# krejciadam/hammock

Measured on AMD Instinct MI355X. Metric: pairwise BLOSUM62 ShiftedScorer scores/sec (all-vs-all, thresholded neighbour list), higher is better.
Workload: dtype u8 (8-bit SWAR lanes, host-proven ranges with 16-bit / literal fallbacks; scores are int32-exact)

## Files before the change

### hammock_amd/_native.py

```python
from __future__ import annotations

import ctypes as C
import os

_HERE = os.path.dirname(os.path.abspath(__file__))
LIB_PATH = os.path.join(_HERE, "lib", "libhammock_hip.so")

HMK_OK = 0
HMK_ERR_BAD_ARG = 1
HMK_ERR_SHIFT_TOO_BIG = 2
HMK_ERR_DEVICE = 3
HMK_ERR_OOM = 4
HMK_ERR_REFERENCE_WOULD_CRASH = 5
HMK_ERR_CAPACITY = 6
HMK_ERR_NO_SEQUENCES = 7
HMK_EDGE_SHARDS = 64
HMK_MAX_LEN = 32
HMK_SURVEY_MAX_BINS = 1024
HMK_PROFILE_SYMBOLS = 21
HMK_PROFILE_MAX_WIDTH = 96
HMK_TARGET_MAX_LEN = 1 << 20
HMK_SCAN_ALL_WINDOWS = 1

SYMBOLS = [
    "hmk_abi_version", "hmk_last_kernel_ms", "hmk_create", "hmk_create_multi", "hmk_device_count", "hmk_destroy", "hmk_last_error", "hmk_set_sequences",
    "hmk_score_pairs_shifted", "hmk_score_with_shift", "hmk_score_pairs_local", "hmk_score_block_shifted", "hmk_score_block_local",
    "hmk_score_pairs_global", "hmk_score_block_global", "hmk_neighbors_global", "hmk_search_global",
    "hmk_neighbors_shifted", "hmk_neighbors_local", "hmk_neighbors_shifted_dev", "hmk_compact_edges_dev", "hmk_pack_rows_dev", "hmk_unpack_rows_dev",
    "hmk_neighbors_last_plan", "hmk_neighbors_last_plan_shared", "hmk_search_shifted", "hmk_search_local", "hmk_search_best_shifted",
    "hmk_assign_shifted", "hmk_assign_local", "hmk_match_clusters_shifted", "hmk_match_clusters_local", "hmk_greedy_continue",
    "hmk_greedy_cluster", "hmk_greedy_from_edges", "hmk_greedy_from_edges_dev", "hmk_greedy_last_phases",
    "hmk_clinkage_cluster", "hmk_clinkage_from_edges", "hmk_set_java_hashset", "hmk_reserve",
    "hmk_cluster_pairs_shifted", "hmk_clinkage_merge", "hmk_clinkage_merge_from_edges",
    "hmk_cluster_linkage_shifted", "hmk_clinkage_split", "hmk_clinkage_split_from_edges",
    "hmk_components_shifted", "hmk_components_from_edges", "hmk_components_from_edges_dev",
    "hmk_cluster_align_shifted", "hmk_score_survey_shifted", "hmk_cluster_separation_shifted",
    "hmk_greedy_sweep", "hmk_greedy_sweep_from_edges", "hmk_greedy_sweep_from_edges_dev",
    "hmk_greedy_orders", "hmk_greedy_orders_from_edges",
    "hmk_representatives_shifted", "hmk_representatives_from_edges", "hmk_representatives_from_edges_dev",
    "hmk_density_shifted", "hmk_density_from_edges", "hmk_density_from_edges_dev",
    "hmk_cluster_profile", "hmk_set_targets", "hmk_scan_shifted",
]


# ... 175 lines not shown
    L.hmk_score_pairs_local.argtypes = [vp, p_u32, p_u32, u64, i32, i32, p_i32]
    L.hmk_score_pairs_global.argtypes = [vp, p_u32, p_u32, u64, i32, i32, p_i32]
    L.hmk_score_with_shift.argtypes = [vp, p_u32, p_u32, u64, i32, i32, p_i32, p_i32]
    L.hmk_score_block_shifted.argtypes = [vp, u32, u32, u32, u32, i32, i32, p_i32]
    L.hmk_score_block_local.argtypes = [vp, u32, u32, u32, u32, i32, i32, p_i32]
    L.hmk_score_block_global.argtypes = [vp, u32, u32, u32, u32, i32, i32, p_i32]
    L.hmk_neighbors_shifted.argtypes = [vp, i32, i32, i32, u32, u32, p_u64, u64, p_u64, C.POINTER(NeighborStats)]
    L.hmk_neighbors_local.argtypes = [vp, i32, i32, i32, u32, u32, p_u64, u64, p_u64, C.POINTER(NeighborStats)]
    L.hmk_neighbors_global.argtypes = [vp, i32, i32, i32, u32, u32, p_u64, u64, p_u64, C.POINTER(NeighborStats)]
    L.hmk_neighbors_shifted_dev.argtypes = [vp, i32, i32, i32, u32, u32, vp, u64, vp, vp]
    L.hmk_compact_edges_dev.argtypes = [vp, vp, u64, vp, vp, u64, vp, vp]
    L.hmk_pack_rows_dev.argtypes = [vp, vp, u64, vp, i32, vp, vp, u64, vp]
    L.hmk_unpack_rows_dev.argtypes = [vp, vp, vp, i32, vp, u64, vp]
    L.hmk_neighbors_last_plan.argtypes = [vp, C.POINTER(NeighborStats)]
    L.hmk_neighbors_last_plan_shared.argtypes = [vp, C.POINTER(C.c_uint32), C.POINTER(C.c_uint32)]
    L.hmk_search_shifted.argtypes = [vp, u32, u32, u32, u32, i32, i32, i32, p_u64, u64, p_u64, C.POINTER(NeighborStats)]
    L.hmk_search_local.argtypes = [vp, u32, u32, u32, u32, i32, i32, i32, p_u64, u64, p_u64, C.POINTER(NeighborStats)]
    L.hmk_search_global.argtypes = [vp, u32, u32, u32, u32, i32, i32, i32, p_u64, u64, p_u64, C.POINTER(NeighborStats)]
    L.hmk_search_best_shifted.argtypes = [vp, u32, u32, u32, u32, i32, i32, i32, u32, p_u32, p_i32, p_u32, C.POINTER(NeighborStats)]
    L.hmk_assign_shifted.argtypes = [vp, u32, u32, u32, u32, p_u32, p_i32, u32, i32, i32, i32, u32, p_u32, p_i32, p_u32,
                                     C.POINTER(NeighborStats)]
    L.hmk_assign_local.argtypes = [vp, u32, u32, u32, u32, p_u32, p_i32, u32, i32, i32, i32, u32, p_u32, p_i32, p_u32,
                                   C.POINTER(NeighborStats)]
    L.hmk_match_clusters_shifted.argtypes = [vp, u32, u32, p_u32, u32, u32, u32, p_u32, p_i32, u32, i32, i32, i32, u32, p_u32, p_i32, p_u32,
                                             C.POINTER(NeighborStats)]
    L.hmk_match_clusters_local.argtypes = [vp, u32, u32, p_u32, u32, u32, u32, p_u32, p_i32, u32, i32, i32, i32, u32, p_u32, p_i32, p_u32,
                                           C.POINTER(NeighborStats)]
    L.hmk_greedy_continue.argtypes = [vp, u32, u32, u32, u32, p_u32, p_i32, u32, i32, i32, i32, p_i32, p_i32, C.POINTER(ContinueStats)]
    L.hmk_greedy_cluster.argtypes = [vp, i32, i32, i32, i32, p_i32, p_i32, p_i32, C.POINTER(GreedyStats)]
    L.hmk_greedy_from_edges_dev.argtypes = [vp, vp, u64, i32, i32, p_i32, p_i32, p_i32, C.POINTER(GreedyStats)]
# ... 54 lines not shown
```

### hammock_amd/api.py

```python
from __future__ import annotations

import ctypes as C

import numpy as np

from . import _native as N

AMINO_ACIDS = "ARNDCQEGHILKMFPSTWYVBZX*"
_NAME_TO_NUM = {c: i for i, c in enumerate(AMINO_ACIDS)}


class HammockException(Exception):
    """HammockException.java"""


class DataException(HammockException):
    """DataException.java -- e.g. "Shift too big" (ShiftedScorer.java:59-62)."""


class FileFormatException(HammockException):
    """FileFormatException.java"""


class DeviceError(HammockException):
# ... 480 lines not shown
            self._raise(st)

    def last_plan(self):
        stats = N.NeighborStats()
        st = N.lib.hmk_neighbors_last_plan(self._h, C.byref(stats))
        if st:
            self._raise(st)
        return stats

    def last_plan_shared(self):
        paired, shared = C.c_uint32(0), C.c_uint32(0)
        st = N.lib.hmk_neighbors_last_plan_shared(self._h, C.byref(paired), C.byref(shared))
        if st:
            self._raise(st)
        return int(paired.value), int(shared.value)

    def greedy_cluster(self, max_shift, shift_penalty, threshold, max_clusters):
        cid = np.full(max(self.n, 1), -1, dtype=np.int32)
        order = np.full(max(self.n, 1), -1, dtype=np.int32)
        self.member_rank = np.zeros(max(self.n, 1), dtype=np.int32)
        stats = N.GreedyStats()
        st = N.lib.hmk_greedy_cluster(self._h, int(max_shift), int(shift_penalty), int(threshold), int(max_clusters),
                                      _ptr(cid, C.c_int32), _ptr(order, C.c_int32),
                                      _ptr(self.member_rank, C.c_int32), C.byref(stats))
        if st:
            self._raise(st, stats)
        return cid[:self.n], order[:stats.n_result_clusters], stats

    def reserve(self, n_sequences):
        st = N.lib.hmk_reserve(self._h, int(n_sequences))
# ... 626 lines not shown
```

### hammock_amd/csrc/hmk_api.cpp

```cpp
#include "hmk_ctx.h"

using namespace hmk::impl;

extern "C" {

int hmk_abi_version(void) { return HMK_ABI_VERSION; }

double hmk_last_kernel_ms(const hmk_ctx *ctx) { return ctx ? ctx->last_kernel_ms : 0.0; }

const char *hmk_last_error(const hmk_ctx *ctx) { return ctx ? ctx->err.c_str() : g_last_error.c_str(); }

int hmk_create(const int32_t *matrix, int device, hmk_ctx **out) {
    if (!matrix || !out) return fail(nullptr, HMK_ERR_BAD_ARG, "hmk_create: null argument");
    *out = nullptr;
    hmk_ctx *ctx = new (std::nothrow) hmk_ctx();
    if (!ctx) return fail(nullptr, HMK_ERR_OOM, "out of memory");
    std::memcpy(ctx->M, matrix, sizeof(ctx->M));
    ctx->min_m = ctx->max_m = matrix[0];
    for (int e = 0; e < 576; e++) {
        ctx->min_m = std::min(ctx->min_m, matrix[e]);
        ctx->max_m = std::max(ctx->max_m, matrix[e]);
        if (matrix[e] != matrix[(e % 24) * 24 + e / 24]) ctx->symmetric = false;
        if (matrix[e] < -1000 || matrix[e] > 1000) {
            delete ctx;
// ... 253 lines not shown
    if (!ctx->plan.valid) return fail(ctx, HMK_ERR_BAD_ARG, "no neighbour pass has been planned yet");
    *stats = ctx->plan.stats;
    return HMK_OK;
}

int hmk_neighbors_last_plan_shared(hmk_ctx *ctx, uint32_t *paired_tiles, uint32_t *run_shared_tiles) {
    if (!ctx || !paired_tiles || !run_shared_tiles) return fail(ctx, HMK_ERR_BAD_ARG, "null argument");
    std::lock_guard<std::mutex> lock(ctx->mu);
    refresh_switches(ctx);
    if (!ctx->plan.valid) return fail(ctx, HMK_ERR_BAD_ARG, "no neighbour pass has been planned yet");
    *paired_tiles = ctx->plan.paired_tiles;
    *run_shared_tiles = ctx->plan.run_shared_tiles;
    return HMK_OK;
}

int hmk_neighbors_shifted(hmk_ctx *ctx, int max_shift, int shift_penalty, int threshold, uint32_t part,
                          uint32_t n_parts, uint64_t *edges, uint64_t capacity, uint64_t *n_edges,
                          hmk_neighbor_stats *stats) {
    if (!ctx) return fail(nullptr, HMK_ERR_BAD_ARG, "null context");
    std::lock_guard<std::mutex> lock(ctx->mu);
    refresh_switches(ctx);
    if (!n_edges) return fail(ctx, HMK_ERR_BAD_ARG, "n_edges must not be null");
    unsigned long long counts[HMK_EDGE_SHARDS];
    double ms = 0;
    int st = neighbors_internal(ctx, max_shift, shift_penalty, threshold, part, n_parts, capacity, counts, &ms);
    if (st) return st;
    const uint64_t total = total_of(counts);
    *n_edges = total;
    if (stats) {
        *stats = ctx->plan.stats;
// ... 280 lines not shown
```

### hammock_amd/csrc/hmk_common.cpp

```cpp
#include <atomic>

#include "hmk_ctx.h"
#include "hmk_grid.h"

namespace hmk {

static std::atomic<int> g_test_grid_cap{0};
void set_test_grid_cap(int cap) { g_test_grid_cap.store(cap < 1 ? 0 : cap, std::memory_order_relaxed); }
uint32_t capped_grid(const char *kernel, uint32_t wanted) {
    const int cap = g_test_grid_cap.load(std::memory_order_relaxed);
    if (cap < 1 || wanted <= (uint32_t)cap) return wanted;
    std::fprintf(stderr, "[hmk grid] %s %u -> %d\n", kernel, wanted, cap);
    return (uint32_t)cap;
}

namespace impl {

thread_local std::string g_last_error;

void Switches::read() {
    auto flag = [](const char *name) { return getenv(name) != nullptr; };
    auto num = [](const char *name, int dflt) { const char *v = getenv(name); return v ? atoi(v) : dflt; };
    *this = Switches();
    greedy_timing = flag("HMK_GREEDY_TIMING");
    no_band = flag("HMK_NO_BAND");
    no_rows_kernel = flag("HMK_NO_ROWS_KERNEL");
    key_sort = flag("HMK_NO_KEY_SORT") ? 0 : num("HMK_KEY_SORT_KEYS", 2) == 1 ? 1 : 2;
    no_row_shared = flag("HMK_NO_ROW_SHARED");
    key_row_pairs = getenv("HMK_KEY_ROW_PAIRS") ? (num("HMK_KEY_ROW_PAIRS", 0) != 0 ? 1 : 0) : -1;
    no_row_run_share = flag("HMK_NO_ROW_RUN_SHARE");
    adj_8byte = flag("HMK_ADJ_8BYTE");
    local_literal = flag("HMK_LOCAL_LITERAL");
    local_signed = flag("HMK_LOCAL_SIGNED");
    local_no_pk = flag("HMK_LOCAL_NO_PK");
    multi_replicate = flag("HMK_MULTI_REPLICATE");
    multi_force_copies = flag("HMK_MULTI_FORCE_COPIES");
    if (const char *v = getenv("HMK_SECOND_LOOP")) second_loop = std::strcmp(v, "device") == 0 ? 1 : 2;
    phase1_threads = std::max(0, num("HMK_PHASE1_THREADS", 0));
    phase1_window = std::max(0, num("HMK_PHASE1_WINDOW", 0));
    if (const char *v = getenv("HMK_PHASE1_HOST_BAND")) {
        host_band_rows = std::max(0, atoi(v));
        if (const char *c = std::strchr(v, ',')) host_band_far_t = std::max(0, atoi(c + 1));
    }
    loop_chain = getenv("HMK_LOOP_CHAIN") ? (num("HMK_LOOP_CHAIN", 0) != 0 ? 1 : 0) : -1;
    loop_passes = std::min(8, std::max(0, num("HMK_LOOP_PASSES", 0)));
// ... 221 lines not shown
```

### hammock_amd/csrc/hmk_ctx.h

```cpp
#ifndef HMK_CTX_H
#define HMK_CTX_H
#include <hip/hip_runtime_api.h>

#include <algorithm>
#include <chrono>
#include <condition_variable>
#include <functional>
#include <future>
#include <memory>
#include <cstdio>
#include <cstdlib>
#include <cstring>
#include <map>
#include <mutex>
#include <numeric>
#include <string>
#include <tuple>
#include <thread>
#include <vector>

#include "hmk_internal.h"
#include "hmk_kernels.h"
#include "hmk_sizing.h"

// ... 68 lines not shown
    SB_SCAN_HITS, SB_SCAN_CNT,
    SB_SCAN_HASH, SB_SCAN_PAIRS, SB_SCAN_COV,
    SB_ORD_EDGES, SB_ORD_STATE, SB_ORD_POS,
    SB_ORD_IDS, SB_ORD_SUPPORT, SB_ORD_PARTNERS,
    SB_N
};

struct Switches {
    bool greedy_timing = false;
    bool no_band = false;
    bool no_rows_kernel = false;
    int key_sort = 2;
    bool no_row_shared = false;
    int key_row_pairs = -1;
    bool no_row_run_share = false;
    bool adj_8byte = false;
    bool local_literal = false;
    bool local_signed = false;
    bool local_no_pk = false;
    bool multi_replicate = false;
    bool multi_force_copies = false;
    int second_loop = 0;
    int phase1_threads = 0, phase1_window = 0;
    int host_band_rows = 0, host_band_far_t = 0;
    int loop_chain = -1;
    int loop_passes = 0;
    int precheck = 0;
    int late_buffers_delay_ms = 0;
    int csr_bucket_shift = 0;
    uint64_t edge_guess = 0;
// ... 14 lines not shown

struct Plan : PlanArrays {
    bool valid = false;
    int X = 0, p = 0, thr = 0;
    uint32_t part = 0, n_parts = 1;
    uint32_t band_rows = 0;
    int64_t band_req = 0;
    int lbmax = 12, lpad = 16;
    bool exact = false;
    bool rows_exact = false;
    bool no_rows_kernel = false;
    int key_sort = 2;
    bool row_shared = true;
    int key_row_pairs = -1;
    bool row_run_share = true;
    bool key_pairs = false;
    uint32_t paired_tiles = 0, run_shared_tiles = 0;
    uint32_t *d_keyrun = nullptr;
    uint32_t *d_keytab = nullptr;
    uint32_t cols_per_tile = 16384;
    uint8_t *d_mb = nullptr;
    std::vector<Group> groups;
    hmk_neighbor_stats stats{};
    uint64_t band_pairs = 0;
    uint32_t q0 = 0, q1 = 0, r0 = 0, r1 = 0;
};

struct PlanLocal : PlanArrays {
    bool valid = false;
    uint32_t part = 0, n_parts = 1;
    bool triangle = false;
    uint32_t n_tiles = 0;
// ... 272 lines not shown
```

### hammock_amd/csrc/hmk_internal.h

```cpp
#ifndef HMK_INTERNAL_H
#define HMK_INTERNAL_H

#include <stdint.h>

#include <functional>
#include <string>
#include <vector>

#include "../../include/hammock_hip.h"

namespace hmk {


enum { PATH_U8 = 0, PATH_U16 = 1, PATH_DIRECT = 2, PATH_ROWS = 3 };

struct TileClass {
    uint8_t la, lb;
    uint8_t nd;
    uint8_t case_b;
    uint8_t x;
    uint8_t path;
    uint8_t nw;
    uint8_t pad;
    int32_t g;
// ... 21 lines not shown
    uint64_t cap_per_shard;
    uint32_t n_tiles;
    uint32_t lpad;
    uint32_t symmetric;
    uint32_t row_is_m;
    uint32_t perm_identity;
    uint32_t *deg;
    uint32_t deg_m_offset;
    const uint32_t *keyrun;
    const uint32_t *keytab;
};

constexpr int KEYTAB_DWORDS = 16;
constexpr int ROWS_KEY_PAIR_GROUPS = 2;
constexpr uint32_t ROWS_RUN_SHARED = 1u << 8;
constexpr bool rows_keyed(int x, int d, int cap, bool exact, int g) { return exact && d == 0 && (g == 1 || g == ROWS_KEY_PAIR_GROUPS) && x == 3 && cap == 12; }
constexpr int rows_key_pos(int x, int l, int q) { return l / 2 - 1 + q < x ? x : l / 2 - 1 + q; }

struct Nbr {
    uint32_t m;
    int32_t s;
    uint32_t id() const { return m; }
    int32_t score() const { return s; }
};
struct NbrPacked {
    uint32_t v;
    uint32_t id() const { return v >> 8; }
    int32_t score() const { return (int32_t)(v & 0xFFu); }
};

// ... 85 lines not shown
```

### hammock_amd/csrc/hmk_kernels.h

```cpp
#ifndef HMK_KERNELS_H
#define HMK_KERNELS_H

#include <hip/hip_runtime_api.h>
#include <stdint.h>

#include "hmk_internal.h"
#include "hmk_scan.h"

namespace hmk {

int swar_rows_per_tile(int lbmax, int nw, bool exact);
int swar_lbmax_for(int lb);

hipError_t launch_neighbors_swar(int lbmax, int nw, bool exact, const NeighborParams &P,
                                 uint32_t tile_base, uint32_t n_tiles, hipStream_t s);
bool rows_kernel_available(int X, int la, int lb, bool exact);
int rows_cap_for(int lb);
int rows_per_tile_rows(int X, int d, int cap, bool exact, bool key_pairs = false);
hipError_t launch_neighbors_rows(int X, int d, int cap, bool exact, const NeighborParams &P, uint32_t tile_base,
                                 uint32_t n_tiles, bool key_pairs, hipStream_t s);
hipError_t warm_neighbors_rows_module();
hipError_t launch_rows_keytab(const uint8_t *res_sorted, uint32_t lpad, uint32_t n, const uint8_t *mb, int case_b, int X, int L,
                              const uint32_t (&cinit)[8], uint32_t *keytab, uint32_t n_groups);
hipError_t launch_neighbors_direct(const NeighborParams &P, uint32_t tile_base, uint32_t n_tiles,
                                   const int32_t *d_matrix, int max_shift, int shift_penalty, int threshold,
                                   hipStream_t s);
hipError_t launch_probe_spin(unsigned long long *when, long long ticks, hipStream_t s);
hipError_t launch_pairs(int scorer, const uint8_t *res32, const uint8_t *len, const int32_t *d_matrix,
                        const uint32_t *pi, const uint32_t *pj, uint64_t n_pairs, uint32_t r0, uint32_t c0,
                        uint32_t width, int a, int b, int32_t *out, int32_t *out_shift, hipStream_t s);

hipError_t launch_neighbors_local(int lbmax, bool enc, bool force_signed, bool force_unpacked, const NeighborParams &P, uint32_t tile_base,
                                  uint32_t n_tiles, const int32_t *d_matrix, int gap_open, int gap_extend, int threshold, hipStream_t s);

hipError_t launch_neighbors_local_literal(const NeighborParams &P, uint32_t tile_base, uint32_t n_tiles, const int32_t *d_matrix,
                                          int gap_open, int gap_extend, int threshold, hipStream_t s);

hipError_t launch_neighbors_global(int lbmax, bool literal, const NeighborParams &P, uint32_t tile_base, uint32_t n_tiles,
// ... 105 lines not shown
```

### hammock_amd/csrc/hmk_plan.cpp

```cpp
#include "hmk_ctx.h"

namespace hmk { namespace impl {

template <class T, class Cmp>
void parallel_stable_sort(std::vector<T> &v, Cmp before) {
    const size_t n = v.size();
    const unsigned hw = usable_cpus();
    size_t runs = 1;
    while (runs < 8 && runs < (hw ? hw : 1u) && n / (2 * runs) >= 32768) runs *= 2;
    if (runs == 1) { std::stable_sort(v.begin(), v.end(), before); return; }
    std::vector<size_t> cut(runs + 1);
    for (size_t r = 0; r <= runs; r++) cut[r] = n * r / runs;
    {
        std::vector<std::thread> pool;
        for (size_t r = 1; r < runs; r++) pool.emplace_back([&, r] { std::stable_sort(v.begin() + (long)cut[r], v.begin() + (long)cut[r + 1], before); });
        std::stable_sort(v.begin(), v.begin() + (long)cut[1], before);
        for (std::thread &th : pool) th.join();
    }
    std::vector<T> other(n);
    std::vector<T> *from = &v, *to = &other;
    for (size_t width = 1; width < runs; width *= 2) {
        std::vector<std::thread> pool;
        for (size_t r = 0; r < runs; r += 2 * width) {
            auto job = [&, r] {
// ... 246 lines not shown
        c.path = u16 ? PATH_U16 : PATH_U8;
        c.g = (int32_t)g;
        const int lpd = u16 ? 2 : 4, bits = u16 ? 16 : 8;
        const int ndw = (nd + lpd - 1) / lpd;
        c.nw = (uint8_t)ndw;
        for (int t = 0; t < nd; t++) c.cinit[t / lpd] |= (uint32_t)ci[t] << ((t % lpd) * bits);
    }
    *out = c;
}

int build_plan(hmk_ctx *ctx, int X, int p, int thr, uint32_t part, uint32_t n_parts, int64_t band_rows, bool key_sort_ok) {
    Plan &pl = ctx->plan;
    const int want_keys = key_sort_ok ? ctx->sw.key_sort : 0;
    if (pl.valid && pl.X == X && pl.p == p && pl.thr == thr && pl.part == part && pl.n_parts == n_parts &&
        (band_rows < 0 || pl.band_req == band_rows) && pl.no_rows_kernel == ctx->sw.no_rows_kernel && pl.key_sort == want_keys &&
        pl.row_shared == !ctx->sw.no_row_shared && pl.key_row_pairs == ctx->sw.key_row_pairs && pl.row_run_share == !ctx->sw.no_row_run_share)
        return HMK_OK;
    free_plan(pl);
    if (band_rows < 0) band_rows = 0;
    const int64_t band_req = band_rows;
    const bool plan_timing = ctx->sw.greedy_timing;
    const auto plan_t0 = std::chrono::steady_clock::now();
    auto plan_lap = [&](const char *what) {
        if (plan_timing)
            fprintf(stderr, "[hmk plan] %s at %.2f ms\n", what,
                    std::chrono::duration<double, std::milli>(std::chrono::steady_clock::now() - plan_t0).count());
    };
    const uint32_t n = ctx->n;
    if (n == 0) return fail(ctx, HMK_ERR_NO_SEQUENCES, "no sequences set (hmk_set_sequences)");
    if (X < 0) return fail(ctx, HMK_ERR_BAD_ARG, "max_shift must be >= 0");
    if (n_parts == 0 || part >= n_parts) return fail(ctx, HMK_ERR_BAD_ARG, "part must be < n_parts");
// ... 76 lines not shown
    pl.rows_exact = false;
    if (use_rows && ctx->min_len == ctx->max_len) {
        TileClass t1;
        classify(ctx, ctx->min_len, ctx->min_len, X, p, thr, &t1);
        pl.rows_exact = (t1.path == PATH_U8 || (refine && all_rows_fit)) && rows_kernel_available(X, ctx->min_len, ctx->min_len, true);
    }
    if (!use_rows && ctx->min_len == 12 && ctx->max_len == 12 && X == 3) {
        TileClass t12;
        classify(ctx, 12, 12, X, p, thr, &t12);
        pl.exact = t12.path == PATH_U8 && t12.nw == 2;
    }
    pl.key_sort = want_keys;
    pl.row_shared = !ctx->sw.no_row_shared;
    pl.key_row_pairs = ctx->sw.key_row_pairs;
    pl.row_run_share = !ctx->sw.no_row_run_share;
    std::vector<uint32_t> keyrun;
    const int L1 = ctx->min_len;
    const bool key_sorted = pl.key_sort > 0 && pl.rows_exact && !(refine && !all_rows_fit) &&
                            rows_keyed(X, 0, L1, true, rows_per_tile_rows(X, 0, L1, true) / 8) && n >= 2;
    if (key_sorted) {
        const int k0 = rows_key_pos(X, L1, 0), k1 = rows_key_pos(X, L1, 1);
        auto key_of = [&](uint32_t k) { return (uint32_t)ctx->res[ctx->off[k] + k0] * HMK_ALPHABET + ctx->res[ctx->off[k] + k1]; };
        const uint32_t b0 = band_end[L1], b1 = bucket[L1 + 1];
        std::vector<uint32_t> cnt(HMK_ALPHABET * HMK_ALPHABET + 1, 0u), sorted(perm.begin() + b0, perm.begin() + b1);
        for (uint32_t q = b0; q < b1; q++) cnt[key_of(perm[q]) + 1]++;
        for (int v = 0; v < HMK_ALPHABET * HMK_ALPHABET; v++) cnt[v + 1] += cnt[v];
        for (uint32_t q = b0; q < b1; q++) sorted[cnt[key_of(perm[q])]++] = perm[q];
        std::copy(sorted.begin(), sorted.end(), perm.begin() + b0);
        keyrun.resize(2 * (size_t)n);
        uint32_t r0 = 0, r01 = 0;
// ... 82 lines not shown
    if (key_sorted && pl.row_shared) {
        const int k0 = rows_key_pos(X, L1, 0), k1 = rows_key_pos(X, L1, 1);
        auto keys_at = [&](uint32_t q) { const uint32_t k = perm[q]; return (uint32_t)ctx->res[ctx->off[k] + k0] << 8 | ctx->res[ctx->off[k] + k1]; };
        for (Tile &t : tiles) {
            for (uint32_t g = 0; 8 * g + 8 <= t.nrows; g++) {
                bool same = true;
                for (uint32_t r = 1; r < 8 && same; r++) same = keys_at(t.row0 + 8 * g + r) == keys_at(t.row0 + 8 * g);
                if (same) t.row_shared |= 1u << g;
            }
            if (pl.key_pairs && pl.row_run_share && t.nrows == 8u * ROWS_KEY_PAIR_GROUPS && (t.row_shared & 3u) == 3u &&
                keys_at(t.row0 + 8) == keys_at(t.row0))
                t.row_shared |= ROWS_RUN_SHARED;
        }
        plan_lap("row-shared groups");
    }
    pl.paired_tiles = pl.key_pairs ? (uint32_t)tiles.size() : 0u;
    pl.run_shared_tiles = 0;
    for (const Tile &t : tiles) pl.run_shared_tiles += (t.row_shared & ROWS_RUN_SHARED) ? 1u : 0u;

    st = upload_plan(ctx, pl, perm, (size_t)pl.lpad, 16, pl.exact ? 8 : 1, classes, tiles);
    if (!st) st = upload_biased_matrix(ctx, pl);
    if (st) return st;
    if (key_sorted) {
        if (classes.size() != 1) return fail(ctx, HMK_ERR_DEVICE, "key-sorted plan with more than one class");
        const uint32_t n_groups = (n + 7) / 8;
        const size_t tab_dwords = (size_t)n_groups * 2 * HMK_ALPHABET * KEYTAB_DWORDS;
        HIPCHK(ctx, hipMalloc((void **)&pl.d_keyrun, keyrun.size() * 4));
        HIPCHK(ctx, hipMemcpy(pl.d_keyrun, keyrun.data(), keyrun.size() * 4, hipMemcpyHostToDevice));
        HIPCHK(ctx, hipMalloc((void **)&pl.d_keytab, tab_dwords * 4));
        HIPCHK(ctx, launch_rows_keytab(pl.d_res_sorted, (uint32_t)pl.lpad, n, pl.d_mb, classes.at(0).case_b, X, L1, classes.at(0).cinit, pl.d_keytab,
                                       n_groups));
        HIPCHK(ctx, hipStreamSynchronize(nullptr));
    }
    pl.X = X; pl.p = p; pl.thr = thr; pl.part = part; pl.n_parts = n_parts;
    pl.valid = true;
    plan_lap("device copies");
    return HMK_OK;
}

static int build_plan_rect(hmk_ctx *ctx, Plan &pl, int X, int p, int thr, uint32_t q0, uint32_t q1, uint32_t r0, uint32_t r1, bool tri) {
    if (pl.valid && pl.X == X && pl.p == p && pl.thr == thr && pl.q0 == q0 && pl.q1 == q1 && pl.r0 == r0 && pl.r1 == r1 &&
        pl.no_rows_kernel == ctx->sw.no_rows_kernel)
        return HMK_OK;
    free_plan(pl);
    if (tri && !ctx->symmetric) return fail(ctx, HMK_ERR_BAD_ARG, "a triangle plan needs a symmetric matrix");
    Buckets bq, br;
// ... 152 lines not shown
```

### hammock_amd/csrc/k_neighbors_rows.h

```cpp
#ifndef HMK_NEIGHBORS_ROWS_H
#define HMK_NEIGHBORS_ROWS_H
#include "hmk_device.h"

namespace hmk {

constexpr int ROWS_STAGE_CAPFORM = 320, ROWS_STAGE_EXACT = 640, ROWS_STAGE_SHORT = 1024;
constexpr int ROWS_INLOOP_MAXCELLS = 45;
constexpr int rows_cells(int x, int cap) { return cap * (2 * x + 1) - x * (x + 1); }
constexpr bool rows_inloop(int x, int cap) { return rows_cells(x, cap) > ROWS_INLOOP_MAXCELLS; }
constexpr bool rows_inloop_shape(int x, int d, int cap, bool exact) { return (exact && d > 0) || rows_inloop(x, cap); }
constexpr int rows_stage(int x, int d, int cap, bool exact) {
    return !exact ? ROWS_STAGE_CAPFORM : rows_inloop_shape(x, d, cap, exact) ? ROWS_STAGE_EXACT : ROWS_STAGE_SHORT;
}
constexpr int rows_groups(int x, int , int cap, bool exact) {
    return !exact ? 2 : rows_inloop(x, cap) ? 1 : 2;
}
constexpr bool rows_two_ended(int x, int d, int cap, bool exact, int g) { return exact && !rows_inloop_shape(x, d, cap, exact) && g == 2; }

template <typename T>
__device__ __forceinline__ T rows_table_read(uint32_t addr) {
    return *reinterpret_cast<const volatile HMK_LDS T *>((uintptr_t)addr);
}
constexpr int rows_waves(int nd, int cap, int lds_bytes, bool exact) {
    const int v = cap + 2 * nd + 36 + (exact ? 0 : 6);
// ... 586 lines not shown
    const Tile T = P.tiles[tile_base + blockIdx.x];
    const TileClass *Cp = P.classes + T.cls;
    const int la = Cp->la;
    int lbs = EXACT_LB ? CAP : (int)Cp->lb;
    const bool case_b = Cp->case_b != 0;
    const int tid = threadIdx.x;
    HMK_LDS uint32_t *stage = (HMK_LDS uint32_t *)stage_all + __builtin_amdgcn_readfirstlane(tid >> 6) * STAGE_CAP;

    constexpr bool KEYED = KEY_FORMS && rows_keyed(X, D, CAP, EXACT_LB, G);
    const bool keyed = KEYED && P.keyrun != nullptr;
    const bool rs_first = keyed && (T.row_shared & 1u) != 0;
    const uint32_t rs_groups = keyed ? T.row_shared : 0u;

    build_begin();
    const uint32_t tab_addr = lds_addr(tab);
    for (int e = tid; e < 576; e += 256) mb[e] = P.mb[e];
    for (int e = tid; e < R * 32; e += 256) {
        const int r = e >> 5, k = e & 31;
        uint8_t v = 0;
        if ((uint32_t)r < T.nrows && (uint32_t)k < P.lpad) v = P.res_sorted[(size_t)(T.row0 + r) * P.lpad + k];
        rowres[e] = v;
    }
    __syncthreads();
    for (int e = tid; e < G * (NI + NEND) * 24 * 2; e += 256) {
        const int h = e & 1, ic = e >> 1;
        const int gi = ic / 24, c = ic - gi * 24;
        const int g = gi / (NI + NEND), k = gi - g * (NI + NEND);
        int i = k < NI ? k : la - 1 - (k - NI);
        const int dst = k < NI ? S::pos_addr(g, k) : S::end_addr(g, k - NI);
        if constexpr (KEYED)
            if ((G == 1 ? rs_first : ((rs_groups >> g) & 1u) != 0) && k == S::key_pos(0) && h == 1) i = S::key_pos(1);
        uint32_t v = 0;
        if (i >= 0 && i < la) {
#pragma unroll
            for (int q = 0; q < 4; q++) {
                const int r = 8 * g + 4 * h + q;
                if ((uint32_t)r < T.nrows) {
                    const int a = rowres[r * 32 + i];
                    v |= (uint32_t)(case_b ? mb[c * 24 + a] : mb[a * 24 + c]) << (q * 8);
                }
            }
        }
        *reinterpret_cast<uint32_t *>(tab + dst + c * 8 + h * 4) = v;
    }
    __syncthreads();
    build_end();

    uint32_t ci[ND];
#pragma unroll
    for (int u = 0; u < ND; u++) ci[u] = ((Cp->cinit[u >> 2] >> ((u & 3) * 8)) & 0xFFu) * 0x01010101u;

    constexpr bool TWO = rows_two_ended(X, D, CAP, EXACT_LB, G);
    uint32_t cnt = 0;
    uint32_t cnt_hi = 0;
    const uint32_t col_end = T.col0 + T.ncols;
    const uint32_t n_batches = (T.ncols + 255) / 256;
    const bool interior = T.diag == 0 && T.ncols % 256 == 0;
    const bool prio = true;

    const uint8_t *const res_sorted = P.res_sorted;
// ... 4 lines not shown
    const uint64_t ka64 = (uint64_t)(uintptr_t)__builtin_amdgcn_kernarg_segment_ptr();
    const uint32_t ka_lo = (uint32_t)ka64, ka_hi = (uint32_t)(ka64 >> 32);
    uint32_t acc[G];
#pragma unroll
    for (int g = 0; g < G; g++) acc[g] = 0;
    static_assert(!KEYED || (G <= 2 && 2 * ND <= KEYTAB_DWORDS), "key table entry; at most two row groups per tile");
    static_assert(!KEYED || (S::body_reads(3, false) == 58 && S::body_reads(1, false) == 65 && S::body_reads(0, false) == 72), "ordinary bodies");
    static_assert(!KEYED || (S::body_reads(3, true) == 54 && S::body_reads(1, true) == 60 && S::body_reads(0, true) == 66), "row-shared bodies (and the lead of a run-shared tile)");
    static_assert(!KEYED || (S::follower_reads(3) == 48 && S::follower_reads(1) == 53 && S::follower_reads(0) == 58), "followers of a run-shared tile");
    static_assert(!KEYED || (S::run_carried_planes(3) == 6 && S::run_carried_planes(1) == 7 && S::run_carried_planes(0) == 7), "dwords a lead hands over");
    static_assert(!KEYED || (S::run_body_adds(3, 2) == 62 && S::run_body_adds(1, 2) == 69 && S::run_body_adds(0, 2) == 75 && S::run_body_adds(3, 3) == 58 &&
                             S::run_body_adds(1, 3) == 64 && S::run_body_adds(0, 3) == 68), "sums of the lead and the follower");
    const uint32_t wave = __builtin_amdgcn_readfirstlane(tid >> 6);
    const uint32_t *kt_tile = nullptr, *kr_wave = nullptr;
    if (keyed) {
        kt_tile = P.keytab + (size_t)(T.row0 >> 3) * (2 * 24 * KEYTAB_DWORDS);
        kr_wave = P.keyrun + 2 * (size_t)(T.col0 + wave * 64);
    }
    auto key_entry = [](const uint32_t *e, uint32_t (&k0)[ND], uint32_t (&k1)[ND]) {
#pragma unroll
        for (int u = 0; u + 1 < ND; u += 2) {
            const u32x4 a = rows_const_load<u32x4>(e + 2 * u);
            k0[u] = a.x; k1[u] = a.y; k0[u + 1] = a.z; k1[u + 1] = a.w;
        }
        if constexpr (ND & 1) {
            const u32x2 a = rows_const_load<u32x2>(e + 2 * (ND - 1));
            k0[ND - 1] = a.x; k1[ND - 1] = a.y;
        }
    };
    using No = std::false_type;
    using Yes = std::true_type;
// ... 12 lines not shown
                ra = rows_const_load<u32x2>(kr_wave);
                const u32x2 rb = rows_const_load<u32x2>(kr_wave + 2 * last);
                if (ra.x == rb.x) kmode = ra.y == rb.y ? 3 : 1;
            }
        }
        uint32_t off[CAP], toff[S::NT];
        S::offsets_of(words, tw, tab_addr, tab_addr, off, toff);
        const bool look = !DEFER || (bt & 3u) == 3u || bt + 1 == n_batches;
        uint32_t Pm[ND];

        if constexpr (RUNS) {
            static_assert(INLOOP && !DEFER && !TWO, "paired tiles: an in-loop shape");
            auto body = [&](auto gt, auto kt, auto rt, uint32_t (&W0)[ND], uint32_t (&W1)[ND]) __attribute__((always_inline)) {
                constexpr int g = decltype(gt)::value, KM = decltype(kt)::value;
                constexpr bool RUN = decltype(rt)::value;
                const uint32_t *const kt_group = kt_tile + (size_t)g * (2 * 24 * KEYTAB_DWORDS);
                [[maybe_unused]] const bool row_shared = (rs_groups & (1u << g)) != 0;
                uint32_t ks0[ND], ks1[ND];
                if constexpr (KM == 3) {
                    uint32_t kb0[ND], kb1[ND];
                    key_entry(kt_group + (ra.x & 31u) * KEYTAB_DWORDS, ks0, ks1);
                    key_entry(kt_group + (24 + (ra.y & 31u)) * KEYTAB_DWORDS, kb0, kb1);
#pragma unroll
                    for (int u = 0; u < ND; u++) { ks0[u] += kb0[u]; ks1[u] += kb1[u]; }
                } else if constexpr (KM == 1) {
                    key_entry(kt_group + (ra.x & 31u) * KEYTAB_DWORDS, ks0, ks1);
#pragma unroll
                    for (int u = 0; u < ND; u++) asm volatile("" : "+s"(ks0[u]), "+s"(ks1[u]));
                }
                const uint32_t (&s0)[ND] = KM != 0 ? ks0 : ci;
                const uint32_t (&s1)[ND] = KM != 0 ? ks1 : ci;
// ... 68 lines not shown
                        uint32_t W0[ND], W1[ND];
                        body(gt, kt, No{}, W0, W1);
                        hits(gt, No{}, W0, W1);
                    });
                }
            };
            if (kmode == 3) both(std::integral_constant<int, 3>{});
            else if (kmode == 1) both(std::integral_constant<int, 1>{});
            else both(std::integral_constant<int, 0>{});
        } else {
            auto one_group = [&](auto gt) {
                constexpr int g = decltype(gt)::value;
                if ((uint32_t)(8 * g) >= T.nrows) return;
                uint32_t W0[ND], W1[ND];
                if constexpr (KEYED) {
                    const uint32_t *const kt_group = kt_tile + (size_t)g * (2 * 24 * KEYTAB_DWORDS);
                    const bool row_shared = G == 1 ? rs_first : (rs_groups & (1u << g)) != 0;
                    uint32_t ks0[ND], ks1[ND];
                    if (kmode == 3) {
                        uint32_t kb0[ND], kb1[ND];
                        key_entry(kt_group + (ra.x & 31u) * KEYTAB_DWORDS, ks0, ks1);
                        key_entry(kt_group + (24 + (ra.y & 31u)) * KEYTAB_DWORDS, kb0, kb1);
#pragma unroll
                        for (int u = 0; u < ND; u++) { ks0[u] += kb0[u]; ks1[u] += kb1[u]; }
                        read_phase_begin(prio);
                        if (RUNS && (rs_groups & ROWS_RUN_SHARED) != 0) S::template accumulate_run<g, 3, (g > 0)>(off, ks0, ks1, W0, W1, Pm);
                        else if (row_shared) S::template accumulate<g, 3, true>(off, toff, lbs, ks0, ks1, W0, W1);
                        else S::template accumulate<g, 3>(off, toff, lbs, ks0, ks1, W0, W1);
                    } else if (kmode == 1) {
                        key_entry(kt_group + (ra.x & 31u) * KEYTAB_DWORDS, ks0, ks1);
#pragma unroll
// ... 131 lines not shown
```

### hammock_amd/csrc/k_neighbors_rows.hip

```cpp
#include "k_rows_shapes.h"

namespace hmk {

int rows_cap_for(int lb) { return lb <= 12 ? 12 : lb <= 16 ? 16 : lb <= 20 ? 20 : 0; }

namespace {
int rows_part_of(int X, int d, int cap, bool exact) {
    if (exact) {
#define HMK_F(PV, XV, L) if (X == XV && d == 0 && cap == L) return PV;
        HMK_ROWS_EXACT_LIST(HMK_F)
#undef HMK_F
        return -1;
    }
#define HMK_C(PV, XV, DV, CAPV) if (X == XV && d == DV && cap == CAPV) return PV;
    HMK_ROWS_CAP_LIST(HMK_C)
#undef HMK_C
    return -1;
}
}

int rows_per_tile_rows(int X, int d, int cap, bool exact, bool key_pairs) {
    if (rows_part_of(X, d, cap, exact) < 0) return 0;
    if (key_pairs) return rows_keyed(X, d, cap, exact, ROWS_KEY_PAIR_GROUPS) ? 8 * ROWS_KEY_PAIR_GROUPS : 0;
    return 8 * rows_groups(X, d, cap, exact);
// ... 25 lines not shown
    if (e >= (uint64_t)n_groups * 2 * HMK_ALPHABET * KEYTAB_DWORDS) return;
    const int d = (int)(e % KEYTAB_DWORDS), c = (int)(e / KEYTAB_DWORDS % HMK_ALPHABET), q = (int)(e / (KEYTAB_DWORDS * HMK_ALPHABET) % 2);
    const uint32_t g = (uint32_t)(e / (2 * HMK_ALPHABET * KEYTAB_DWORDS));
    const int u = d >> 1, h = d & 1, i = rows_key_pos(X, L, q) + u - X;
    uint32_t v = 0;
    if (u <= 2 * X && i >= 0 && i < L) {
        for (int t = 0; t < 4; t++) {
            const uint32_t r = 8 * g + 4 * h + t;
            if (r < n) {
                const int a = res_sorted[(size_t)r * lpad + i];
                v |= (uint32_t)(case_b ? mb[c * HMK_ALPHABET + a] : mb[a * HMK_ALPHABET + c]) << (8 * t);
            }
        }
    }
    if (q == 0 && u <= 2 * X) v += ((cinit.w[u >> 2] >> ((u & 3) * 8)) & 0xFFu) * 0x01010101u;
    keytab[e] = v;
}

hipError_t launch_rows_keytab(const uint8_t *res_sorted, uint32_t lpad, uint32_t n, const uint8_t *mb, int case_b, int X, int L,
                              const uint32_t (&cinit)[8], uint32_t *keytab, uint32_t n_groups) {
    const uint64_t total = (uint64_t)n_groups * 2 * HMK_ALPHABET * KEYTAB_DWORDS;
    if (total == 0) return hipSuccess;
    KeytabInit ci;
    for (int k = 0; k < 8; k++) ci.w[k] = cinit[k];
    hipLaunchKernelGGL(k_rows_keytab, dim3((unsigned)((total + 255) / 256)), dim3(256), 0, nullptr, res_sorted, lpad, n, mb, case_b, X, L, ci,
                       keytab, n_groups);
    return hipGetLastError();
}

}
```

### include/hammock_hip.h

```cpp
#ifndef HAMMOCK_HIP_H
#define HAMMOCK_HIP_H

#include <stdint.h>

#ifdef __cplusplus
extern "C" {
#endif

#define HMK_ABI_VERSION 4
#define HMK_ALPHABET 24
#define HMK_MAX_LEN 32
#define HMK_MAX_SEQUENCES (1u << 24)
#define HMK_EDGE_SHARDS 64

typedef enum {
    HMK_OK = 0,
    HMK_ERR_BAD_ARG = 1,
    HMK_ERR_SHIFT_TOO_BIG = 2,
    HMK_ERR_DEVICE = 3,
    HMK_ERR_OOM = 4,
    HMK_ERR_REFERENCE_WOULD_CRASH = 5,
    HMK_ERR_CAPACITY = 6,
    HMK_ERR_NO_SEQUENCES = 7
} hmk_status;
// ... 56 lines not shown
int hmk_neighbors_global(hmk_ctx *ctx, int gap_open, int gap_extend, int threshold, uint32_t part,
                         uint32_t n_parts, uint64_t *edges, uint64_t capacity, uint64_t *n_edges,
                         hmk_neighbor_stats *stats);

int hmk_neighbors_shifted_dev(hmk_ctx *ctx, int max_shift, int shift_penalty, int threshold,
                              uint32_t part, uint32_t n_parts, void *d_edges, uint64_t capacity,
                              void *d_counts, void *stream);
int hmk_compact_edges_dev(hmk_ctx *ctx, const void *d_edges, uint64_t capacity, const void *d_counts,
                          void *d_out, uint64_t out_capacity, void *d_total, void *stream);
int hmk_pack_rows_dev(hmk_ctx *ctx, const void *d_edges, uint64_t capacity, const void *d_counts, int threshold,
                      void *d_row_start, void *d_adj, uint64_t adj_capacity, void *stream);
int hmk_unpack_rows_dev(hmk_ctx *ctx, const void *d_row_start, const void *d_adj, int threshold, void *d_edges_out,
                        uint64_t out_capacity, void *stream);
int hmk_neighbors_last_plan(hmk_ctx *ctx, hmk_neighbor_stats *stats);
int hmk_neighbors_last_plan_shared(hmk_ctx *ctx, uint32_t *paired_tiles, uint32_t *run_shared_tiles);


int hmk_search_shifted(hmk_ctx *ctx, uint32_t q0, uint32_t q1, uint32_t r0, uint32_t r1,
                       int max_shift, int shift_penalty, int threshold,
                       uint64_t *edges, uint64_t capacity, uint64_t *n_edges, hmk_neighbor_stats *stats);
int hmk_search_local(hmk_ctx *ctx, uint32_t q0, uint32_t q1, uint32_t r0, uint32_t r1,
                     int gap_open, int gap_extend, int threshold,
                     uint64_t *edges, uint64_t capacity, uint64_t *n_edges, hmk_neighbor_stats *stats);
int hmk_search_global(hmk_ctx *ctx, uint32_t q0, uint32_t q1, uint32_t r0, uint32_t r1,
                      int gap_open, int gap_extend, int threshold,
                      uint64_t *edges, uint64_t capacity, uint64_t *n_edges, hmk_neighbor_stats *stats);
int hmk_search_best_shifted(hmk_ctx *ctx, uint32_t q0, uint32_t q1, uint32_t r0, uint32_t r1,
                            int max_shift, int shift_penalty, int threshold, uint32_t k,
                            uint32_t *hit_index, int32_t *hit_score, uint32_t *n_hits,
                            hmk_neighbor_stats *stats);
// ... 441 lines not shown
```

Before: 2642 billion.

## Precompute per-tile row score tables at plan time and load them into LDS

Adds a plan-time kernel that builds each 8-row group's per-position substitution-score LDS table (including the row-shared key substitution) and stores it interleaved with the existing key table in global memory. In the keyed plain-edges rows kernel, tiles flagged with the new table bit copy the prebuilt table into LDS with vector loads, instead of rebuilding it from the score matrix and residues in every tile. This is meant to remove the per-tile table build cost. In exchange it uses more global memory, changes the keytab stride, and only applies when the minimum length is 12. An env switch can disable it.

```diff
diff --git a/hammock_amd/_native.py b/hammock_amd/_native.py
--- a/hammock_amd/_native.py
+++ b/hammock_amd/_native.py
@@ -27,7 +27,7 @@
     "hmk_score_pairs_shifted", "hmk_score_with_shift", "hmk_score_pairs_local", "hmk_score_block_shifted", "hmk_score_block_local",
     "hmk_score_pairs_global", "hmk_score_block_global", "hmk_neighbors_global", "hmk_search_global",
     "hmk_neighbors_shifted", "hmk_neighbors_local", "hmk_neighbors_shifted_dev", "hmk_compact_edges_dev", "hmk_pack_rows_dev", "hmk_unpack_rows_dev",
-    "hmk_neighbors_last_plan", "hmk_neighbors_last_plan_shared", "hmk_search_shifted", "hmk_search_local", "hmk_search_best_shifted",
+    "hmk_neighbors_last_plan", "hmk_neighbors_last_plan_shared", "hmk_neighbors_last_plan_tables", "hmk_search_shifted", "hmk_search_local", "hmk_search_best_shifted",
     "hmk_assign_shifted", "hmk_assign_local", "hmk_match_clusters_shifted", "hmk_match_clusters_local", "hmk_greedy_continue",
     "hmk_greedy_cluster", "hmk_greedy_from_edges", "hmk_greedy_from_edges_dev", "hmk_greedy_last_phases",
     "hmk_clinkage_cluster", "hmk_clinkage_from_edges", "hmk_set_java_hashset", "hmk_reserve",
@@ -233,6 +233,7 @@
     L.hmk_unpack_rows_dev.argtypes = [vp, vp, vp, i32, vp, u64, vp]
     L.hmk_neighbors_last_plan.argtypes = [vp, C.POINTER(NeighborStats)]
     L.hmk_neighbors_last_plan_shared.argtypes = [vp, C.POINTER(C.c_uint32), C.POINTER(C.c_uint32)]
+    L.hmk_neighbors_last_plan_tables.argtypes = [vp, C.POINTER(C.c_uint32), C.POINTER(C.c_uint64)]
     L.hmk_search_shifted.argtypes = [vp, u32, u32, u32, u32, i32, i32, i32, p_u64, u64, p_u64, C.POINTER(NeighborStats)]
     L.hmk_search_local.argtypes = [vp, u32, u32, u32, u32, i32, i32, i32, p_u64, u64, p_u64, C.POINTER(NeighborStats)]
     L.hmk_search_global.argtypes = [vp, u32, u32, u32, u32, i32, i32, i32, p_u64, u64, p_u64, C.POINTER(NeighborStats)]
diff --git a/hammock_amd/api.py b/hammock_amd/api.py
--- a/hammock_amd/api.py
+++ b/hammock_amd/api.py
@@ -518,6 +518,13 @@
         if st:
             self._raise(st)
         return int(paired.value), int(shared.value)
+
+    def last_plan_tables(self):
+        tiles, nbytes = C.c_uint32(0), C.c_uint64(0)
+        st = N.lib.hmk_neighbors_last_plan_tables(self._h, C.byref(tiles), C.byref(nbytes))
+        if st:
+            self._raise(st)
+        return int(tiles.value), int(nbytes.value)
 
     def greedy_cluster(self, max_shift, shift_penalty, threshold, max_clusters):
         cid = np.full(max(self.n, 1), -1, dtype=np.int32)
diff --git a/hammock_amd/csrc/hmk_api.cpp b/hammock_amd/csrc/hmk_api.cpp
--- a/hammock_amd/csrc/hmk_api.cpp
+++ b/hammock_amd/csrc/hmk_api.cpp
@@ -291,6 +291,16 @@
     return HMK_OK;
 }
 
+int hmk_neighbors_last_plan_tables(hmk_ctx *ctx, uint32_t *table_tiles, uint64_t *table_bytes) {
+    if (!ctx || !table_tiles || !table_bytes) return fail(ctx, HMK_ERR_BAD_ARG, "null argument");
+    std::lock_guard<std::mutex> lock(ctx->mu);
+    refresh_switches(ctx);
+    if (!ctx->plan.valid) return fail(ctx, HMK_ERR_BAD_ARG, "no neighbour pass has been planned yet");
+    *table_tiles = ctx->plan.table_tiles;
+    *table_bytes = ctx->plan.table_bytes;
+    return HMK_OK;
+}
+
 int hmk_neighbors_shifted(hmk_ctx *ctx, int max_shift, int shift_penalty, int threshold, uint32_t part,
                           uint32_t n_parts, uint64_t *edges, uint64_t capacity, uint64_t *n_edges,
                           hmk_neighbor_stats *stats) {
diff --git a/hammock_amd/csrc/hmk_common.cpp b/hammock_amd/csrc/hmk_common.cpp
--- a/hammock_amd/csrc/hmk_common.cpp
+++ b/hammock_amd/csrc/hmk_common.cpp
@@ -29,6 +29,7 @@
     no_row_shared = flag("HMK_NO_ROW_SHARED");
     key_row_pairs = getenv("HMK_KEY_ROW_PAIRS") ? (num("HMK_KEY_ROW_PAIRS", 0) != 0 ? 1 : 0) : -1;
     no_row_run_share = flag("HMK_NO_ROW_RUN_SHARE");
+    no_tile_tables = flag("HMK_NO_TILE_TABLES");
     adj_8byte = flag("HMK_ADJ_8BYTE");
     local_literal = flag("HMK_LOCAL_LITERAL");
     local_signed = flag("HMK_LOCAL_SIGNED");
diff --git a/hammock_amd/csrc/hmk_ctx.h b/hammock_amd/csrc/hmk_ctx.h
--- a/hammock_amd/csrc/hmk_ctx.h
+++ b/hammock_amd/csrc/hmk_ctx.h
@@ -106,6 +106,7 @@
     bool no_row_shared = false;
     int key_row_pairs = -1;
     bool no_row_run_share = false;
+    bool no_tile_tables = false;
     bool adj_8byte = false;
     bool local_literal = false;
     bool local_signed = false;
@@ -150,8 +151,11 @@
     bool row_shared = true;
     int key_row_pairs = -1;
     bool row_run_share = true;
+    bool tile_tables = true;
     bool key_pairs = false;
     uint32_t paired_tiles = 0, run_shared_tiles = 0;
+    uint32_t table_tiles = 0;
+    uint64_t table_bytes = 0;
     uint32_t *d_keyrun = nullptr;
     uint32_t *d_keytab = nullptr;
     uint32_t cols_per_tile = 16384;
diff --git a/hammock_amd/csrc/hmk_internal.h b/hammock_amd/csrc/hmk_internal.h
--- a/hammock_amd/csrc/hmk_internal.h
+++ b/hammock_amd/csrc/hmk_internal.h
@@ -59,6 +59,11 @@
 constexpr int KEYTAB_DWORDS = 16;
 constexpr int ROWS_KEY_PAIR_GROUPS = 2;
 constexpr uint32_t ROWS_RUN_SHARED = 1u << 8;
+constexpr uint32_t ROWS_TILE_TABLE = 1u << 9;
+constexpr int ROWTAB_POSITIONS = 12;
+constexpr int ROWTAB_DWORDS = ROWTAB_POSITIONS * 24 * 2;
+constexpr int KEYGROUP_KEY_DWORDS = 2 * 24 * KEYTAB_DWORDS;
+constexpr int KEYGROUP_DWORDS = KEYGROUP_KEY_DWORDS + ROWTAB_DWORDS;
 constexpr bool rows_keyed(int x, int d, int cap, bool exact, int g) { return exact && d == 0 && (g == 1 || g == ROWS_KEY_PAIR_GROUPS) && x == 3 && cap == 12; }
 constexpr int rows_key_pos(int x, int l, int q) { return l / 2 - 1 + q < x ? x : l / 2 - 1 + q; }
 
diff --git a/hammock_amd/csrc/hmk_kernels.h b/hammock_amd/csrc/hmk_kernels.h
--- a/hammock_amd/csrc/hmk_kernels.h
+++ b/hammock_amd/csrc/hmk_kernels.h
@@ -22,6 +22,8 @@
 hipError_t warm_neighbors_rows_module();
 hipError_t launch_rows_keytab(const uint8_t *res_sorted, uint32_t lpad, uint32_t n, const uint8_t *mb, int case_b, int X, int L,
                               const uint32_t (&cinit)[8], uint32_t *keytab, uint32_t n_groups);
+hipError_t launch_rows_rowtab(const uint8_t *res_sorted, uint32_t lpad, uint32_t n, const uint8_t *mb, int case_b, int X, int L,
+                              bool row_shared, uint32_t *keytab, uint32_t n_groups);
 hipError_t launch_neighbors_direct(const NeighborParams &P, uint32_t tile_base, uint32_t n_tiles,
                                    const int32_t *d_matrix, int max_shift, int shift_penalty, int threshold,
                                    hipStream_t s);
diff --git a/hammock_amd/csrc/hmk_plan.cpp b/hammock_amd/csrc/hmk_plan.cpp
--- a/hammock_amd/csrc/hmk_plan.cpp
+++ b/hammock_amd/csrc/hmk_plan.cpp
@@ -284,7 +284,8 @@
     const int want_keys = key_sort_ok ? ctx->sw.key_sort : 0;
     if (pl.valid && pl.X == X && pl.p == p && pl.thr == thr && pl.part == part && pl.n_parts == n_parts &&
         (band_rows < 0 || pl.band_req == band_rows) && pl.no_rows_kernel == ctx->sw.no_rows_kernel && pl.key_sort == want_keys &&
-        pl.row_shared == !ctx->sw.no_row_shared && pl.key_row_pairs == ctx->sw.key_row_pairs && pl.row_run_share == !ctx->sw.no_row_run_share)
+        pl.row_shared == !ctx->sw.no_row_shared && pl.key_row_pairs == ctx->sw.key_row_pairs && pl.row_run_share == !ctx->sw.no_row_run_share &&
+        pl.tile_tables == !ctx->sw.no_tile_tables)
         return HMK_OK;
     free_plan(pl);
     if (band_rows < 0) band_rows = 0;
@@ -391,6 +392,7 @@
     pl.row_shared = !ctx->sw.no_row_shared;
     pl.key_row_pairs = ctx->sw.key_row_pairs;
     pl.row_run_share = !ctx->sw.no_row_run_share;
+    pl.tile_tables = !ctx->sw.no_tile_tables;
     std::vector<uint32_t> keyrun;
     const int L1 = ctx->min_len;
     const bool key_sorted = pl.key_sort > 0 && pl.rows_exact && !(refine && !all_rows_fit) &&
@@ -503,6 +505,11 @@
         }
         plan_lap("row-shared groups");
     }
+    const bool tile_tables = key_sorted && pl.tile_tables && L1 == ROWTAB_POSITIONS;
+    if (tile_tables)
+        for (Tile &t : tiles) t.row_shared |= ROWS_TILE_TABLE;
+    pl.table_tiles = tile_tables ? (uint32_t)tiles.size() : 0u;
+    pl.table_bytes = tile_tables ? (uint64_t)((n + 7) / 8) * ROWTAB_DWORDS * 4 : 0u;
     pl.paired_tiles = pl.key_pairs ? (uint32_t)tiles.size() : 0u;
     pl.run_shared_tiles = 0;
     for (const Tile &t : tiles) pl.run_shared_tiles += (t.row_shared & ROWS_RUN_SHARED) ? 1u : 0u;
@@ -513,12 +520,15 @@
     if (key_sorted) {
         if (classes.size() != 1) return fail(ctx, HMK_ERR_DEVICE, "key-sorted plan with more than one class");
         const uint32_t n_groups = (n + 7) / 8;
-        const size_t tab_dwords = (size_t)n_groups * 2 * HMK_ALPHABET * KEYTAB_DWORDS;
+        const size_t tab_dwords = (size_t)n_groups * KEYGROUP_DWORDS;
         HIPCHK(ctx, hipMalloc((void **)&pl.d_keyrun, keyrun.size() * 4));
         HIPCHK(ctx, hipMemcpy(pl.d_keyrun, keyrun.data(), keyrun.size() * 4, hipMemcpyHostToDevice));
         HIPCHK(ctx, hipMalloc((void **)&pl.d_keytab, tab_dwords * 4));
         HIPCHK(ctx, launch_rows_keytab(pl.d_res_sorted, (uint32_t)pl.lpad, n, pl.d_mb, classes.at(0).case_b, X, L1, classes.at(0).cinit, pl.d_keytab,
                                        n_groups));
+        if (tile_tables)
+            HIPCHK(ctx, launch_rows_rowtab(pl.d_res_sorted, (uint32_t)pl.lpad, n, pl.d_mb, classes.at(0).case_b, X, L1, pl.row_shared, pl.d_keytab,
+                                           n_groups));
         HIPCHK(ctx, hipStreamSynchronize(nullptr));
     }
     pl.X = X; pl.p = p; pl.thr = thr; pl.part = part; pl.n_parts = n_parts;
diff --git a/hammock_amd/csrc/k_neighbors_rows.h b/hammock_amd/csrc/k_neighbors_rows.h
--- a/hammock_amd/csrc/k_neighbors_rows.h
+++ b/hammock_amd/csrc/k_neighbors_rows.h
@@ -624,6 +624,19 @@
 
     build_begin();
     const uint32_t tab_addr = lds_addr(tab);
+    constexpr bool TABLED = KEYED && MODE == EDGES_PLAIN;
+    static_assert(!TABLED || (S::GROUP_STEP == ROWTAB_DWORDS * 4 && TAB_BYTES == G * ROWTAB_DWORDS * 4 && NEND == 0), "the plan's tile table is the LDS table of one group");
+    if (TABLED && keyed && (T.row_shared & ROWS_TILE_TABLE) != 0) {
+        constexpr int PIECES = ROWTAB_DWORDS / 4;
+        const uint32_t *const rt_tile = P.keytab + (size_t)(T.row0 >> 3) * KEYGROUP_DWORDS + KEYGROUP_KEY_DWORDS;
+        for (int e = tid; e < G * PIECES; e += 256) {
+            const int g = e / PIECES, q = e - g * PIECES;
+            u32x4 v = {0, 0, 0, 0};
+            if ((uint32_t)(8 * g) < T.nrows) v = *reinterpret_cast<const u32x4 *>(rt_tile + (size_t)g * KEYGROUP_DWORDS + 4 * q);
+            *reinterpret_cast<u32x4 *>(tab + 16 * e) = v;
+        }
+        __syncthreads();
+    } else {
     for (int e = tid; e < 576; e += 256) mb[e] = P.mb[e];
     for (int e = tid; e < R * 32; e += 256) {
         const int r = e >> 5, k = e & 31;
@@ -654,6 +667,7 @@
         *reinterpret_cast<uint32_t *>(tab + dst + c * 8 + h * 4) = v;
     }
     __syncthreads();
+    }
     build_end();
 
     uint32_t ci[ND];
@@ -688,7 +702,7 @@
     const uint32_t wave = __builtin_amdgcn_readfirstlane(tid >> 6);
     const uint32_t *kt_tile = nullptr, *kr_wave = nullptr;
     if (keyed) {
-        kt_tile = P.keytab + (size_t)(T.row0 >> 3) * (2 * 24 * KEYTAB_DWORDS);
+        kt_tile = P.keytab + (size_t)(T.row0 >> 3) * KEYGROUP_DWORDS;
         kr_wave = P.keyrun + 2 * (size_t)(T.col0 + wave * 64);
     }
     auto key_entry = [](const uint32_t *e, uint32_t (&k0)[ND], uint32_t (&k1)[ND]) {
@@ -731,7 +745,7 @@
             auto body = [&](auto gt, auto kt, auto rt, uint32_t (&W0)[ND], uint32_t (&W1)[ND]) __attribute__((always_inline)) {
                 constexpr int g = decltype(gt)::value, KM = decltype(kt)::value;
                 constexpr bool RUN = decltype(rt)::value;
-                const uint32_t *const kt_group = kt_tile + (size_t)g * (2 * 24 * KEYTAB_DWORDS);
+                const uint32_t *const kt_group = kt_tile + (size_t)g * KEYGROUP_DWORDS;
                 [[maybe_unused]] const bool row_shared = (rs_groups & (1u << g)) != 0;
                 uint32_t ks0[ND], ks1[ND];
                 if constexpr (KM == 3) {
@@ -830,7 +844,7 @@
                 if ((uint32_t)(8 * g) >= T.nrows) return;
                 uint32_t W0[ND], W1[ND];
                 if constexpr (KEYED) {
-                    const uint32_t *const kt_group = kt_tile + (size_t)g * (2 * 24 * KEYTAB_DWORDS);
+                    const uint32_t *const kt_group = kt_tile + (size_t)g * KEYGROUP_DWORDS;
                     const bool row_shared = G == 1 ? rs_first : (rs_groups & (1u << g)) != 0;
                     uint32_t ks0[ND], ks1[ND];
                     if (kmode == 3) {
diff --git a/hammock_amd/csrc/k_neighbors_rows.hip b/hammock_amd/csrc/k_neighbors_rows.hip
--- a/hammock_amd/csrc/k_neighbors_rows.hip
+++ b/hammock_amd/csrc/k_neighbors_rows.hip
@@ -63,7 +63,35 @@
         }
     }
     if (q == 0 && u <= 2 * X) v += ((cinit.w[u >> 2] >> ((u & 3) * 8)) & 0xFFu) * 0x01010101u;
-    keytab[e] = v;
+    keytab[(size_t)g * KEYGROUP_DWORDS + e % KEYGROUP_KEY_DWORDS] = v;
+}
+
+__global__ void __launch_bounds__(256) k_rows_rowtab(const uint8_t *__restrict__ res_sorted, uint32_t lpad, uint32_t n,
+                                                     const uint8_t *__restrict__ mb, int case_b, int X, int L, int row_shared,
+                                                     uint32_t *__restrict__ keytab, uint32_t n_groups) {
+    const uint64_t e = (uint64_t)blockIdx.x * 256 + threadIdx.x;
+    if (e >= (uint64_t)n_groups * ROWTAB_DWORDS) return;
+    const uint32_t g = (uint32_t)(e / ROWTAB_DWORDS);
+    const int d = (int)(e % ROWTAB_DWORDS), h = d & 1, c = (d >> 1) % HMK_ALPHABET, k = d / (2 * HMK_ALPHABET);
+    const int k0 = rows_key_pos(X, L, 0), k1 = rows_key_pos(X, L, 1);
+    int i = k;
+    if (row_shared && k == k0 && h == 1 && 8 * g + 8 <= n) {
+        const uint8_t *first = res_sorted + (size_t)(8 * g) * lpad;
+        bool same = true;
+        for (int r = 1; r < 8; r++) same = same && first[(size_t)r * lpad + k0] == first[k0] && first[(size_t)r * lpad + k1] == first[k1];
+        if (same) i = k1;
+    }
+    uint32_t v = 0;
+    if (i < L) {
+        for (int t = 0; t < 4; t++) {
+            const uint32_t r = 8 * g + 4 * h + t;
+            if (r < n) {
+                const int a = res_sorted[(size_t)r * lpad + i];
+                v |= (uint32_t)(case_b ? mb[c * HMK_ALPHABET + a] : mb[a * HMK_ALPHABET + c]) << (8 * t);
+            }
+        }
+    }
+    keytab[(size_t)g * KEYGROUP_DWORDS + KEYGROUP_KEY_DWORDS + d] = v;
 }
 
 hipError_t launch_rows_keytab(const uint8_t *res_sorted, uint32_t lpad, uint32_t n, const uint8_t *mb, int case_b, int X, int L,
@@ -77,4 +105,14 @@
     return hipGetLastError();
 }
 
+hipError_t launch_rows_rowtab(const uint8_t *res_sorted, uint32_t lpad, uint32_t n, const uint8_t *mb, int case_b, int X, int L,
+                              bool row_shared, uint32_t *keytab, uint32_t n_groups) {
+    const uint64_t total = (uint64_t)n_groups * ROWTAB_DWORDS;
+    if (total == 0) return hipSuccess;
+    if (L != ROWTAB_POSITIONS) return hipErrorInvalidValue;
+    hipLaunchKernelGGL(k_rows_rowtab, dim3((unsigned)((total + 255) / 256)), dim3(256), 0, nullptr, res_sorted, lpad, n, mb, case_b, X, L,
+                       row_shared ? 1 : 0, keytab, n_groups);
+    return hipGetLastError();
 }
+
+}
diff --git a/include/hammock_hip.h b/include/hammock_hip.h
--- a/include/hammock_hip.h
+++ b/include/hammock_hip.h
@@ -94,6 +94,7 @@
                         uint64_t out_capacity, void *stream);
 int hmk_neighbors_last_plan(hmk_ctx *ctx, hmk_neighbor_stats *stats);
 int hmk_neighbors_last_plan_shared(hmk_ctx *ctx, uint32_t *paired_tiles, uint32_t *run_shared_tiles);
+int hmk_neighbors_last_plan_tables(hmk_ctx *ctx, uint32_t *table_tiles, uint64_t *table_bytes);
 
 
 int hmk_search_shifted(hmk_ctx *ctx, uint32_t q0, uint32_t q1, uint32_t r0, uint32_t r1,
```

After: 2678 billion (median of 6 runs). +1.3%, better.
